# jackbaggins/RayTracing2-fork

Hardware: AMD Instinct MI355X
Metric: Msamples/sec at 1920×1080 Cornell+OBJ; per-pixel RMSE vs CPU ref (higher is better)
Workload: dtype f32

## Files before the change

raytracing2-fork_amd/csrc/device/rt2_k5_resident.h:

```cpp
#pragma once

extern "C" __device__ int rt2_writelane(int value, int lane, int old) __asm("llvm.amdgcn.writelane.i32");

namespace {

constexpr int kResGroups = 38;

struct K5Resident {
    h8 rec[kResGroups * 4 * 64];
};

template <MfmaSpec S>
__device__ __forceinline__ bool exact_group(unsigned long long M, int G, int n_tris, cfloat* tri, const f3& o,
                                            const f3& d, float& best, int& bi, float& bestK, MfmaDiag& dg) {
    if constexpr (S.diag) dg.hot += 1;
    uint32_t m32 = (uint32_t)(M | M >> 32);
    const float bk0 = bestK;
    while (m32) {
        const int tt = __builtin_ctz(m32);
        m32 &= m32 - 1;
        const int idx = 32 * G + tt;
        if (idx >= n_tris) break;
        if constexpr (S.diag) dg.exact += 1;
        cfloat* tp = tri + 12 * idx;
// ... 170 lines not shown
    }
    if constexpr (S.diag) xl_counts(dg, pairs, pairs, (tested + 31) >> 5);
    if (more && __ballot(bestK != bk0)) {
        if constexpr (S.diag) tc = __builtin_amdgcn_s_memtime();
        rebuild();
        if constexpr (S.diag) dg.t_pub += __builtin_amdgcn_s_memtime() - tc;
    }
}

template <MfmaSpec S>
__device__ __forceinline__ void phase_prio(int phase) {
    if constexpr (S.phase_prio > 0) {
        const bool hi = (S.phase_prio == 1 && phase == 0) || (S.phase_prio == 2 && phase == 1) ||
                        (S.phase_prio == 3 && phase == 2) || (S.phase_prio == 4 && phase != 0);
        if (hi)
            __builtin_amdgcn_s_setprio(1);
        else
            __builtin_amdgcn_s_setprio(0);
    }
}

struct ClusterDiag {
    unsigned long long skipped = 0, one = 0, two = 0, rays = 0;
};

__device__ __forceinline__ h8 cluster_rows_frag(const h8* a0, unsigned long long need) {
    typedef uint32_t u4 __attribute__((ext_vector_type(4)));
    const int l = (int)lane_id();
    const int c0 = __popc((uint32_t)need), c1 = __popc((uint32_t)(need >> 32));
    const int rk = (int)lanes_below(need);
    const bool nb = (need >> l) & 1ull;
    const int rest = ((l - rk) + (l < 32 ? c0 : c1 + 2 * c0)) & 31;
    const uint32_t row = (uint32_t)(nb ? rk : rest);
    const auto sw = __builtin_amdgcn_permlane32_swap(row, row, false, false);
    const int half = l & 32;
    const int to0 = 4 * ((int)sw[0] + half), to1 = 4 * ((int)sw[1] + half);
    const u4 b0 = __builtin_bit_cast(u4, a0[0]), b1 = __builtin_bit_cast(u4, a0[1]);
    const bool first = (l & 31) < c0;
    u4 r;
#pragma unroll
    for (int k = 0; k < 4; k++) {
        const int x0 = __builtin_amdgcn_ds_permute(to0, (int)b0[k]);
        const int x1 = __builtin_amdgcn_ds_permute(to1, (int)b1[k]);
        r[k] = (uint32_t)(first ? x0 : x1);
    }
    return __builtin_bit_cast(h8, r);
}

template <MfmaSpec S>
__device__ __forceinline__ bool sweep_kt_res(const RenderParams& p, const h8* rec, const f3& o, const f3& d,
                                             float& best, int& bi, float& bestK, MfmaDiag& dg, bool upper,
                                             unsigned long long act = 0, ClusterDiag* cd = nullptr) {
    const int lane = (int)lane_id();
    [[maybe_unused]] unsigned long long tc = 0, tsw = 0;
    if constexpr (S.diag) tsw = tc = __builtin_amdgcn_s_memtime();
    auto stamp = [&](unsigned long long& acc) {
        if constexpr (S.diag) {
            const unsigned long long t = __builtin_amdgcn_s_memtime();
            acc += t - tc;
            tc = t;
        }
    };
    const f3 m = cross(d, o);
    MfmaScale sc;
    if (!mfma_scale<true>(p.mfma_A, o, d, m, sc)) return false;
    h8 a0[2], y1[2];
    _Float16 tw16;
    kt_frags<S.kt_lane_w>(d, m, sc, a0, tw16);
    constexpr bool per_group = S.exact_win == 1 && !S.y_skip_last && !S.diag;
// ... 86 lines not shown
                            }
                        }
                        auto one_block = [&](const h8& af, int j, int j1) {
                            for (; j + 1 < j1; j += 2) {
                                const h8* t = tb;
                                unsigned long long M0, M1;
                                kt_group_one2(af, t[0], t[64], t[128], t[kKtOps * 64], t[kKtOps * 64 + 64],
                                              t[kKtOps * 64 + 128], M0, M1);
                                const uint32_t m0 = (uint32_t)(M0 | M0 >> 32), m1 = (uint32_t)(M1 | M1 >> 32);
                                maskv = rt2_writelane((int)m0, j, maskv);
                                maskv = rt2_writelane((int)m1, j + 1, maskv);
                                any |= m0 | m1;
                                tb += 2 * kKtOps * 64;
                            }
                            if (j < j1) {
                                const h8 b0 = tb[0], b1 = tb[64], b2 = tb[128], b3 = {};
                                const unsigned long long M = kt_group<false>(&af, y1, b0, b1, b2, b3, false);
                                const uint32_t m32 = (uint32_t)(M | M >> 32);
                                maskv = rt2_writelane((int)m32, j, maskv);
                                any |= m32;
                                tb += kKtOps * 64;
                            }
                        };
#pragma nounroll
                        for (int k = 0; k < ncl; k++) {
                            const int g0 = __float_as_int(ct[8 * k + 3]), gf = __float_as_int(ct[8 * k + 7]);
                            const int g1 = gf & 0xffff;
                            const unsigned long long need =
                                (unsigned long long)(uint32_t)__builtin_amdgcn_readlane(maskv, kNeedLane + 2 * k) |
                                (unsigned long long)(uint32_t)__builtin_amdgcn_readlane(maskv, kNeedLane + 2 * k + 1) << 32;
                            const int c = __popcll(need);
                            const bool compact = (gf & RT2_CLUSTER_COMPACT) != 0;
                            if constexpr (S.diag)
                                if (compact) {
                                    cd->rays += (unsigned long long)c;
                                    if (!c)
                                        cd->skipped += 1;
                                    else if (!upper || c <= 32)
                                        cd->one += 1;
                                    else
                                        cd->two += 1;
                                }
                            if (!c) {
                                tb += (g1 - g0) * (kKtOps * 64);
                                continue;
                            }
                            if (upper && !(compact && c <= 32)) {
                                int up = 1;
                                asm volatile("" : "+s"(up));
                                two_block(g0, g1, up != 0);
                            } else {
                                h8 af = a0[0];
                                if (upper) af = cluster_rows_frag(a0, need);
                                one_block(af, g0, g1);
                            }
                        }
                        maskv = lane < kNeedLane ? maskv : 0;
                    }
                }
            } else {
                for (int j = 0; j < cnt; j++) {
                    const h8 b0 = tb[0], b1 = tb[64], b2 = tb[128];
                    h8 b3 = {};
                    if constexpr (YP) b3 = tb[192];
                    tb += kKtOps * 64;
                    const unsigned long long M = kt_group<YP>(a0, y1, b0, b1, b2, b3, upper);
                    const uint32_t m32 = (uint32_t)(M | M >> 32);
                    if constexpr (W > 1) maskv = lane == j ? (int)m32 : maskv;
                    any |= m32;
// ... 239 lines not shown
        if (lane_id() == 0) {
            atomicAdd(p.seg_counter + 1, dg.groups);
            atomicAdd(p.seg_counter + 2, dg.hot);
            atomicAdd(p.seg_counter + 3, dg.exact);
            atomicAdd(p.seg_counter + 12, dg.t_wait);
            atomicAdd(p.seg_counter + 13, dg.t_filt);
            atomicAdd(p.seg_counter + 14, dg.t_exact);
            atomicAdd(p.seg_counter + 15, dg.t_swp);
            atomicAdd(p.seg_counter + 16, __builtin_amdgcn_s_memtime() - wl_c0);
            atomicAdd(p.seg_counter + 17, dg.t_issue);
            atomicAdd(p.seg_counter + 18, dg.t_pub);
            atomicAdd(p.seg_counter + 19, dg.claims);
            atomicAdd(p.seg_counter + 7, dg.xl[0]);
            atomicAdd(p.seg_counter + 8, dg.xl[1]);
            atomicAdd(p.seg_counter + 9, dg.xl[2]);
            atomicMax(p.seg_counter + 10, dg.xl[3]);
            atomicAdd(p.seg_counter + 22, pds.d.new_ray);
            atomicAdd(p.seg_counter + 23, pds.d.new_px);
            if constexpr (S.cluster_rows) {
                atomicAdd(p.seg_counter + 24, cdg.skipped);
                atomicAdd(p.seg_counter + 25, cdg.one);
                atomicAdd(p.seg_counter + 26, cdg.two);
                atomicAdd(p.seg_counter + 27, cdg.rays);
            }
        }
}

}
```

raytracing2-fork_amd/csrc/device/rt2_mfma.h:

```cpp
#pragma once

namespace {

typedef _Float16 h8 __attribute__((ext_vector_type(8)));
typedef float f4v __attribute__((ext_vector_type(4)));
typedef float f16v __attribute__((ext_vector_type(16)));

constexpr int kMfmaQ = 5;
constexpr float kMfmaC = 1.0009765625f;
constexpr float kMfmaTs = 0x1p-12f;
constexpr float kMfmaB = 2.0f;

struct MfmaSpec {
    int block;
    int waves;
    int tail_lanes;
    bool diag = false;
    int tile_groups = 0;
    bool fair_prio = false;
    int phase_prio = 0;
    bool flow_prio = false;
    bool kt_lane_w = false;
    bool lean = false;
    bool res_l2 = false;
    int exact_win = 1;
    bool y_skip_last = false;
    bool y_first = false;
    bool exact_lanes = false;
    bool pair_loop = false;
    bool cam_park = false;
    bool cluster_rows = false;
};

struct MfmaDiag {
    unsigned long long groups = 0, hot = 0, exact = 0;
    unsigned long long xl[4] = {};
    unsigned long long t_wait = 0, t_filt = 0, t_exact = 0, t_swp = 0;
    unsigned long long unused1 = 0;
    unsigned long long t_issue = 0, t_pub = 0, claims = 0;
};

struct MfmaCoef {
    double c[kMfmaQ][10];
    double tau;
};
__device__ __forceinline__ void mfma_coefs(const float4* tri, int i, int n, MfmaCoef& k, uint32_t* flags) {
    for (int q = 0; q < kMfmaQ; q++)
        for (int c = 0; c < 10; c++) k.c[q][c] = 0.0;
    k.tau = 1.0;
    if (i >= n) {
        k.c[3][9] = 0x1p13;
        return;
    }
    const float4 t0 = tri[3 * i], t1 = tri[3 * i + 1], t2 = tri[3 * i + 2];
// ... 422 lines not shown
#pragma unroll
    for (int i = 0; i < 16; i++)
        t0[i] = __builtin_amdgcn_bitop3_b32(__float_as_int(U0[i]), __float_as_int(V0[i]), __float_as_int(X0[i]), 0x80);
    const f16v U1 = __builtin_amdgcn_mfma_f32_32x32x16_f16(a, bu1, zero, 0, 0, 0);
#pragma unroll
    for (int i = 0; i < 8; i++) acc0 = __builtin_amdgcn_bitop3_b32(t0[2 * i], t0[2 * i + 1], acc0, 0xFE);
    const f16v V1 = __builtin_amdgcn_mfma_f32_32x32x16_f16(a, bv1, zero, 0, 0, 0);
    const f16v X1 = __builtin_amdgcn_mfma_f32_32x32x16_f16(a, bx1, zero, 0, 0, 0);
#pragma unroll
    for (int i = 0; i < 16; i++)
        t1[i] = __builtin_amdgcn_bitop3_b32(__float_as_int(U1[i]), __float_as_int(V1[i]), __float_as_int(X1[i]), 0x80);
#pragma unroll
    for (int i = 0; i < 8; i++) acc1 = __builtin_amdgcn_bitop3_b32(t1[2 * i], t1[2 * i + 1], acc1, 0xFE);
    __builtin_amdgcn_sched_group_barrier(0x008, 3, 0);
    __builtin_amdgcn_sched_group_barrier(0x002, 16, 0);
    __builtin_amdgcn_sched_group_barrier(0x008, 1, 0);
    __builtin_amdgcn_sched_group_barrier(0x002, 8, 0);
    __builtin_amdgcn_sched_group_barrier(0x008, 2, 0);
    __builtin_amdgcn_sched_group_barrier(0x002, 24, 0);
    M0 = __ballot(acc0 < 0);
    M1 = __ballot(acc1 < 0);
}

__device__ __forceinline__ bool sweep_k16(const RenderParams& p, MfmaK16LaneLds& sh, const f3& o, const f3& d,
                                          float& best, int& bi, float& bestK, bool upper) {
    const int lane = (int)lane_id();
    const int r32 = lane & 31, hl = lane >> 5;
    const f3 m = cross(d, o);
    MfmaScale sc;
    if (!mfma_scale<false>(p.mfma_A, o, d, m, sc)) return false;
    mfma_main_row(&sh.ray[lane][0], d, m, o, sc.sigma);
    const float vz = m.z * sc.sigma;
    const _Float16 hz = (_Float16)vz;
    const _Float16 lz = (_Float16)(vz - (float)hz);
    const float zhi = wave_max(fabsf((float)hz));
    const float zlo = wave_max(fabsf((float)lz));
    auto write_y = [&](float bkv) {
        _Float16 s[16];
        mfma_y_chunk(s, d, o, bkv, sc.sigma, sc.Bmax);
        h8* row = reinterpret_cast<h8*>(&sh.ray[lane][32]);
        row[0] = h8{s[0], s[1], s[2], s[3], s[4], s[5], s[6], s[7]};
        row[1] = h8{s[8], s[9], s[10], s[11], s[12], s[13], s[14], s[15]};
    };
    write_y(bestK);
    __builtin_amdgcn_fence(__ATOMIC_RELEASE, "wavefront");
    __builtin_amdgcn_wave_barrier();
// ... 245 lines not shown
    ri[1] = sc.sigma;
    ri[2] = sc.Tw;
    ri[3] = sc.Bmax;
    ri[4] = m.x;
    ri[5] = m.y;
    ri[6] = m.z;
    ri[7] = bestK;
    if (!ok) return;
    mfma_main_row(&sh.ray[lane][0], d, m, o, sc.sigma);
    {
        _Float16 s[16];
        mfma_y_chunk(s, d, o, bestK, sc.sigma, sc.Bmax);
        for (int j = 0; j < 16; j++) sh.ray[lane][32 + j] = s[j];
    }
    __syncthreads();
    for (int j = 0; j < 48; j++) frags[ray * 80 + j] = sh.ray[lane][j];
    const size_t ray0 = (size_t)blockIdx.x * 64;
    if constexpr (kPerm) {
        const int r32 = lane & 31, hl = lane >> 5;
        h8 a0[2], y1[2];
        [[maybe_unused]] ThrBits tb = {};
        [[maybe_unused]] _Float16 tw16 = (_Float16)0.0f;
        if constexpr (kKthr) {
            kt_frags<LAYOUT == 6>(d, m, sc, a0, tw16);
            kt_y(d, o, bestK, sc, tw16, y1);
        } else {
            _Float16 s[18];
            mfma_main_half_slots(s, d, m, sc.sigma);
            frag_pair(s, a0);
            _Float16 t[16];
            mfma_y_chunk(t, d, o, bestK, sc.sigma, sc.Bmax);
            frag_pair(t, y1);
            const float vz = m.z * sc.sigma;
            const _Float16 hz = (_Float16)vz;
            const _Float16 lz = (_Float16)(vz - (float)hz);
            tb = mfma_thr_bits(sc.Tw, wave_max(fabsf((float)lz)), wave_max(fabsf((float)hz)));
        }
        for (int R = 0; R < 2; R++)
            for (int j = 0; j < 8; j++) {
                frags[(ray0 + 32 * R + r32) * 80 + 48 + 8 * hl + j] = a0[R][j];
                frags[(ray0 + 32 * R + r32) * 80 + 64 + 8 * hl + j] = y1[R][j];
            }
        const h8* fg = reinterpret_cast<const h8*>(kKthr ? p.mfma_kt_frag : p.mfma_k16_frag) + lane;
        const int nops = kKthr ? kKtOps : kK16Ops;
        const f16v zero = {};
        for (int G = 0; G < n_pad / 32; G++) {
            h8 b[kK16Ops];
            for (int op = 0; op < nops; op++) b[op] = fg[(size_t)G * nops * 64 + 64 * op];
            for (int R = 0; R < 2; R++) {
                K16Terms q;
                if constexpr (kKthr) {
                    q.U = __builtin_amdgcn_mfma_f32_32x32x16_f16(a0[R], b[0], zero, 0, 0, 0);
                    q.V = __builtin_amdgcn_mfma_f32_32x32x16_f16(a0[R], b[1], zero, 0, 0, 0);
                    q.X = __builtin_amdgcn_mfma_f32_32x32x16_f16(a0[R], b[2], zero, 0, 0, 0);
                    q.T = zero;
                    q.Y = __builtin_amdgcn_mfma_f32_32x32x16_f16(y1[R], b[3], zero, 0, 0, 0);
                } else {
                    const f16v c = __builtin_amdgcn_mfma_f32_32x32x16_f16(mfma_thr_frag(tb), b[6], zero, 0, 0, 0);
                    q.U = __builtin_amdgcn_mfma_f32_32x32x16_f16(a0[R], b[0], c, 0, 0, 0);
                    q.V = __builtin_amdgcn_mfma_f32_32x32x16_f16(a0[R], b[2], c, 0, 0, 0);
                    q.X = __builtin_amdgcn_mfma_f32_32x32x16_f16(a0[R], b[4], c, 0, 0, 0);
                    q.T = c;
                    q.Y = __builtin_amdgcn_mfma_f32_32x32x16_f16(y1[R], b[6], c, 0, 0, 0);
                }
                for (int i = 0; i < 16; i++) {
                    const size_t rr = ray0 + 32 * R + 8 * (i >> 2) + 4 * hl + (i & 3);
                    float* tt = terms + (rr * n_pad + 32 * G + r32) * 5;
                    tt[0] = q.U[i];
// ... 80 lines not shown
```

raytracing2-fork_amd/csrc/device/rt2_render.hip:

```cpp
#include <hip/hip_runtime.h>

#include <algorithm>
#include <cstdio>
#include <cstdlib>
#include <cstring>
#include <mutex>
#include <string>
#include <type_traits>
#include <vector>

#include "../../../include/rt2.h"
#include "../../../include/rt2_cluster.h"
#include "rt2_math.h"

using namespace rt2d;

#include "rt2_sweep.h"
#include "rt2_path.h"
#include "rt2_brute.h"
#include "rt2_mfma.h"
#include "rt2_k5_tiles.h"
#include "rt2_k5_resident.h"
#include "rt2_assist.h"
#include "rt2_bvh.h"
// ... 368 lines not shown
        HIPCHECK(hipMalloc(&s->d_mfma_k16, (size_t)n_pad32 * kK16Ops * 16 * sizeof(_Float16)));
        HIPCHECK(hipMalloc(&s->d_mfma_k16_tau, (size_t)n_pad32 * sizeof(float)));
        HIPCHECK(hipMalloc(&s->d_mfma_k16_bnd, (size_t)n_pad32 * sizeof(float2)));
        uint32_t* d_mflags = reinterpret_cast<uint32_t*>(s->d_counters + kCounters - 2);
        HIPCHECK(hipMemset(d_mflags, 0, 2 * sizeof(uint32_t)));
        hipLaunchKernelGGL(prep_mfma_k16, dim3((n_pad32 + 255) / 256), dim3(256), 0, 0, s->d_tri, n_tris, n_pad32,
                           s->d_mfma_k16, s->d_mfma_k16_tau, s->d_mfma_k16_bnd, d_mflags);
        HIPCHECK(hipGetLastError());
        uint32_t mflags[2];
        HIPCHECK(hipMemcpy(mflags, d_mflags, sizeof(mflags), hipMemcpyDeviceToHost));
        HIPCHECK(hipMemset(d_mflags, 0, 2 * sizeof(uint32_t)));
        std::memcpy(&s->mfma_A, &mflags[1], sizeof(float));
        s->mfma_ok = s->mfma_A <= 0x1p20f;
        const size_t kt_bytes = (size_t)n_pad32 * kKtOps * 16 * sizeof(_Float16);
        if (n_pad32 / 32 <= kResGroups && rt2_cluster_table_build(tris, n_tris, &s->clusters) < 0) return -1;
        HIPCHECK(hipMalloc(&s->d_mfma_kt, kt_bytes + sizeof(s->clusters)));
        HIPCHECK(hipMemcpy(reinterpret_cast<char*>(s->d_mfma_kt) + kt_bytes, &s->clusters, sizeof(s->clusters),
                           hipMemcpyHostToDevice));
        hipLaunchKernelGGL(prep_mfma_kt, dim3((n_pad32 + 255) / 256), dim3(256), 0, 0, s->d_tri, n_tris, n_pad32,
                           s->d_mfma_kt, d_mflags);
        HIPCHECK(hipGetLastError());
        HIPCHECK(hipDeviceSynchronize());
        HIPCHECK(hipMemset(d_mflags, 0, 2 * sizeof(uint32_t)));
    }
    HIPCHECK(hipDeviceSynchronize());
    return 0;
}

static int ensure_mfma16(rt2_scene* s) {
    if (s->d_mfma || s->n_tris <= 0) return 0;
    HIPCHECK(hipSetDevice(s->device));
    const int n_pad = (s->n_tris + 15) / 16 * 16;
    HIPCHECK(hipMalloc(&s->d_mfma, (size_t)n_pad * kMfmaQ * 32 * sizeof(_Float16)));
    HIPCHECK(hipMalloc(&s->d_mfma_tau, (size_t)n_pad * sizeof(float)));
    HIPCHECK(hipDeviceSynchronize());
    uint32_t* d_mflags = reinterpret_cast<uint32_t*>(s->d_counters + kCounters - 2);
    HIPCHECK(hipMemset(d_mflags, 0, 2 * sizeof(uint32_t)));
    hipLaunchKernelGGL(prep_mfma, dim3((n_pad + 255) / 256), dim3(256), 0, 0, s->d_tri, s->n_tris, n_pad, s->d_mfma,
                       s->d_mfma_tau, d_mflags);
    HIPCHECK(hipGetLastError());
    HIPCHECK(hipMemset(d_mflags, 0, 2 * sizeof(uint32_t)));
    HIPCHECK(hipDeviceSynchronize());
    return 0;
}

extern "C" void rt2_scene_destroy(rt2_scene* s) {
// ... 101 lines not shown
}
#ifdef RT2_EXPERIMENTS
constexpr MfmaSpec kt_yw(MfmaSpec x) {
    x.y_first = true;
    return x;
}
#endif
constexpr MfmaSpec kt_xl(MfmaSpec x) {
    x.exact_lanes = true;
    return x;
}
constexpr MfmaSpec kt_pair(MfmaSpec x) {
    x.pair_loop = true;
    return x;
}
constexpr MfmaSpec kt_park(MfmaSpec x) {
    x.cam_park = true;
    return x;
}
constexpr MfmaSpec kt_cr(MfmaSpec x) {
    x.cluster_rows = true;
    return x;
}
constexpr int kResWin = 38;
constexpr int kResL2Groups = 256;
constexpr MfmaSpec kt_tiles_flow() {
    return MfmaSpec{.block = 768, .waves = 3, .tail_lanes = 0, .tile_groups = 19, .flow_prio = true, .kt_lane_w = true};
}
constexpr MfmaSpec kt_tiles_flow4() {
    MfmaSpec x = kt_tiles_flow();
    x.block = 1024;
    x.waves = 4;
    x.lean = true;
    return x;
}
constexpr Bvh3Spec kBvhDefault{.block = 256, .thresh = 16, .slab = Slab::Markstein, .waves = 5, .diag = false};

#ifdef RT2_EXPERIMENTS
constexpr SmemSpec smem_x(int g, Filter f, Tail t, int lanes, int w, bool stats = false) {
    return SmemSpec{.block = 256, .group = g, .filter = f, .tail = t, .tail_lanes = lanes, .waves = w, .stats = stats};
}
constexpr SplitSpec split_x(int s, Filter f, int w) {
    return SplitSpec{.waves_per_ray = s, .group = 8, .filter = f, .waves = w};
}
constexpr Bvh3Spec bvh3_x(int t, Slab sl, int w, bool diag = false) {
    return Bvh3Spec{.block = 256, .thresh = t, .slab = sl, .waves = w, .diag = diag};
}
#endif

constexpr Variant kVariants[] = {
    RT2_VARIANT(0, K_SMEM, render_smem<kSmemDefault>, 256, "smem/256/max3f8/coop32/w6/lockstep"),
    RT2_VARIANT(109, K_BVH4, render_bvh4<kBvhDefault>, 256, "bvh4/256/t16/w5"),
    RT2_VARIANT(86, K_TILED, render_tiled<kTiledLarge>, 512, "tiled/512/max3f4"),
    RT2_VARIANT(92, K_ASSIST, render_assist<kAssist12>, 768, "assist12/max3f8/w6"),
    RT2_VARIANT(136, K_SMEM, render_smem<kSmemDefault>, 256, "smem/256/max3f8/coop32/w6/lockstep"),
    RT2_VARIANT(227, K_MFMA, render_mfma<kMfmaK5>, 256, "mfma/256/k5/coop8/w3/imax/minred/ymma/t12/llds/ser4/cmp"),
    RT2_VARIANT(353, K_MFMA, render_mfma_k5r<kt_cr(kt_park(kt_pair(kt_xl(kt_win(kt_res(false, false, true, 4), kResWin)))))>, 1024, "mfmar/1024/kt4/res38/coop4/w4/cmp/dpp/lean/lw/pp4", kResGroups),
    RT2_VARIANT(354, K_MFMA, render_mfma_k5r<kt_cr(kt_park(kt_pair(kt_xl(kt_win(kt_res(false, true, true), kResWin)))))>, 1024, "mfmar/1024/kt4/res38/coop4/w4/cmp/fair/dpp/lean/lw", kResGroups),
    RT2_VARIANT(355, K_MFMA, render_mfma_k5r<kt_win(kt_res(true, false, true, 4), kResWin)>, 1024, "mfmarl2/1024/kt4/res38l2/coop4/w4/cmp/dpp/lean/lw/pp4", kResL2Groups),
    RT2_VARIANT(356, K_MFMA, render_mfma_k5r<kt_win(kt_res(true, true, true), kResWin)>, 1024, "mfmarl2/1024/kt4/res38l2/coop4/w4/cmp/fair/dpp/lean/lw", kResL2Groups),
    RT2_VARIANT(380, K_MFMA, render_mfma_k5t<kt_tiles_flow4()>, 1024, "mfmat5/1024/kt4/tile19/coop0/w4/cmp/regs/perm/lw/flowp/lean"),
#ifdef RT2_EXPERIMENTS
    RT2_VARIANT(342, K_MFMA, render_mfma_k5r<kt_win(kt_res(false, false, false), kResWin)>, 1024, "mfmar/1024/kt4/res38/coop4/w4/cmp/dpp/lean", kResGroups),
    RT2_VARIANT(344, K_MFMA, render_mfma_k5r<kt_win(kt_res(false, true, false), kResWin)>, 1024, "mfmar/1024/kt4/res38/coop4/w4/cmp/fair/dpp/lean", kResGroups),
    RT2_VARIANT(345, K_MFMA, render_mfma_k5r<kt_win(kt_res(true, false, false), kResWin)>, 1024, "mfmarl2/1024/kt4/res38l2/coop4/w4/cmp/dpp/lean", kResL2Groups),
    RT2_VARIANT(346, K_MFMA, render_mfma_k5r<kt_win(kt_res(true, true, false), kResWin)>, 1024, "mfmarl2/1024/kt4/res38l2/coop4/w4/cmp/fair/dpp/lean", kResL2Groups),
    RT2_VARIANT(387, K_MFMA, render_mfma_k5r<kt_win(kt_res(false, false, true, 1), kResWin)>, 1024, "mfmar/1024/kt4/res38/coop4/w4/cmp/dpp/lean/lw/pp1", kResGroups),
    RT2_VARIANT(388, K_MFMA, render_mfma_k5r<kt_win(kt_res(false, false, true, 2), kResWin)>, 1024, "mfmar/1024/kt4/res38/coop4/w4/cmp/dpp/lean/lw/pp2", kResGroups),
    RT2_VARIANT(389, K_MFMA, render_mfma_k5r<kt_win(kt_res(false, false, true, 3), kResWin)>, 1024, "mfmar/1024/kt4/res38/coop4/w4/cmp/dpp/lean/lw/pp3", kResGroups),
    RT2_VARIANT(391, K_MFMA, render_mfma_k5r<kt_win(kt_res(false, false, true), kResWin)>, 1024, "mfmar/1024/kt4/res38/coop4/w4/cmp/dpp/lean/lw", kResGroups),
    RT2_VARIANT(350, K_MFMA, render_mfma_k5r<kt_win(kt_res(false, false, true, 0, true), kResWin)>, 1024, "mfmar/1024/kt4/res38/coop4/w4/cmp/diag/dpp/lean/lw", kResGroups),
    RT2_VARIANT(390, K_MFMA, render_mfma_k5r<kt_win(kt_res(false, false, true, 0, true), 1)>, 1024, "mfmar/1024/kt4/res38/coop4/w4/cmp/diag/dpp/lean/lw/xw1", kResGroups),
    RT2_VARIANT(392, K_MFMA, render_mfma_k5r<kt_win(kt_res(false, false, true, 4), 1)>, 1024, "mfmar/1024/kt4/res38/coop4/w4/cmp/dpp/lean/lw/pp4/xw1", kResGroups),
    RT2_VARIANT(393, K_MFMA, render_mfma_k5r<kt_win(kt_res(false, false, true, 4), 1, true)>, 1024, "mfmar/1024/kt4/res38/coop4/w4/cmp/dpp/lean/lw/pp4/xw1s", kResGroups),
    RT2_VARIANT(394, K_MFMA, render_mfma_k5r<kt_win(kt_res(false, false, true, 4), 2)>, 1024, "mfmar/1024/kt4/res38/coop4/w4/cmp/dpp/lean/lw/pp4/xw2", kResGroups),
    RT2_VARIANT(395, K_MFMA, render_mfma_k5r<kt_win(kt_res(false, false, true, 4), 4)>, 1024, "mfmar/1024/kt4/res38/coop4/w4/cmp/dpp/lean/lw/pp4/xw4", kResGroups),
    RT2_VARIANT(396, K_MFMA, render_mfma_k5r<kt_win(kt_res(false, false, true, 4), 8)>, 1024, "mfmar/1024/kt4/res38/coop4/w4/cmp/dpp/lean/lw/pp4/xw8", kResGroups),
    RT2_VARIANT(399, K_MFMA, render_mfma_k5r<kt_win(kt_res(false, false, true, 4), 19)>, 1024, "mfmar/1024/kt4/res38/coop4/w4/cmp/dpp/lean/lw/pp4/xw19", kResGroups),
    RT2_VARIANT(397, K_MFMA, render_mfma_k5r<kt_win(kt_res(true, false, true, 4), 1)>, 1024, "mfmarl2/1024/kt4/res38l2/coop4/w4/cmp/dpp/lean/lw/pp4/xw1", kResL2Groups),
    RT2_VARIANT(398, K_MFMA, render_mfma_k5r<kt_win(kt_res(false, true, true), 1)>, 1024, "mfmar/1024/kt4/res38/coop4/w4/cmp/fair/dpp/lean/lw/xw1", kResGroups),
    RT2_VARIANT(351, K_MFMA, render_mfma_k5r<kt_yw(kt_win(kt_res(false, false, true, 4), kResWin))>, 1024, "mfmar/1024/kt4/res38/coop4/w4/cmp/dpp/lean/lw/pp4/yw", kResGroups),
    RT2_VARIANT(352, K_MFMA, render_mfma_k5r<kt_yw(kt_win(kt_res(true, false, true, 4), kResWin))>, 1024, "mfmarl2/1024/kt4/res38l2/coop4/w4/cmp/dpp/lean/lw/pp4/yw", kResL2Groups),
    RT2_VARIANT(357, K_MFMA, render_mfma_k5r<kt_yw(kt_win(kt_res(false, false, true, 0, true), kResWin))>, 1024, "mfmar/1024/kt4/res38/coop4/w4/cmp/diag/dpp/lean/lw/yw", kResGroups),
    RT2_VARIANT(400, K_MFMA, render_mfma_k5r<kt_win(kt_res(false, false, true, 4), kResWin)>, 1024, "mfmar/1024/kt4/res38/coop4/w4/cmp/dpp/lean/lw/pp4/xwave", kResGroups),
    RT2_VARIANT(401, K_MFMA, render_mfma_k5r<kt_xl(kt_win(kt_res(true, false, true, 4), kResWin))>, 1024, "mfmarl2/1024/kt4/res38l2/coop4/w4/cmp/dpp/lean/lw/pp4/xl", kResL2Groups),
    RT2_VARIANT(402, K_MFMA, render_mfma_k5r<kt_xl(kt_win(kt_res(false, false, true, 0, true), kResWin))>, 1024, "mfmar/1024/kt4/res38/coop4/w4/cmp/diag/dpp/lean/lw/xl", kResGroups),
    RT2_VARIANT(403, K_MFMA, render_mfma_k5r<kt_win(kt_res(false, true, true), kResWin)>, 1024, "mfmar/1024/kt4/res38/coop4/w4/cmp/fair/dpp/lean/lw/xwave", kResGroups),
    RT2_VARIANT(404, K_MFMA, render_mfma_k5r<kt_xl(kt_win(kt_res(true, true, true), kResWin))>, 1024, "mfmarl2/1024/kt4/res38l2/coop4/w4/cmp/fair/dpp/lean/lw/xl", kResL2Groups),
    RT2_VARIANT(405, K_MFMA, render_mfma_k5r<kt_xl(kt_win(kt_res(false, false, true, 4), kResWin))>, 1024, "mfmar/1024/kt4/res38/coop4/w4/cmp/dpp/lean/lw/pp4/nopair/nopark", kResGroups),
    RT2_VARIANT(406, K_MFMA, render_mfma_k5r<kt_pair(kt_xl(kt_win(kt_res(false, false, true, 4), kResWin)))>, 1024, "mfmar/1024/kt4/res38/coop4/w4/cmp/dpp/lean/lw/pp4/nopark", kResGroups),
    RT2_VARIANT(407, K_MFMA, render_mfma_k5r<kt_park(kt_xl(kt_win(kt_res(false, false, true, 4), kResWin)))>, 1024, "mfmar/1024/kt4/res38/coop4/w4/cmp/dpp/lean/lw/pp4/nopair", kResGroups),
    RT2_VARIANT(408, K_MFMA, render_mfma_k5r<kt_xl(kt_win(kt_res(false, true, true), kResWin))>, 1024, "mfmar/1024/kt4/res38/coop4/w4/cmp/fair/dpp/lean/lw/nopair/nopark", kResGroups),
    RT2_VARIANT(409, K_MFMA, render_mfma_k5r<kt_park(kt_pair(kt_xl(kt_win(kt_res(false, false, true, 4), kResWin))))>, 1024, "mfmar/1024/kt4/res38/coop4/w4/cmp/dpp/lean/lw/pp4/nocr", kResGroups),
    RT2_VARIANT(410, K_MFMA, render_mfma_k5r<kt_park(kt_pair(kt_xl(kt_win(kt_res(false, true, true), kResWin))))>, 1024, "mfmar/1024/kt4/res38/coop4/w4/cmp/fair/dpp/lean/lw/nocr", kResGroups),
    RT2_VARIANT(411, K_MFMA, render_mfma_k5r<kt_cr(kt_pair(kt_xl(kt_win(kt_res(false, false, true, 0, true), kResWin))))>, 1024, "mfmar/1024/kt4/res38/coop4/w4/cmp/diag/dpp/lean/lw/xl/cr", kResGroups),
    RT2_VARIANT(370, K_MFMA, render_mfma_k5t<kt_tiles_flow()>, 768, "mfmat5/768/kt4/tile19/coop0/w3/cmp/regs/perm/lw/flowp"),
    RT2_VARIANT(368, K_MFMA, render_mfma_k5t<[] { MfmaSpec x = kt_tiles_flow(); x.diag = true; return x; }()>, 768, "mfmat5/768/kt4/tile19/coop0/w3/cmp/regs/perm/lw/flowp/diag"),
    RT2_VARIANT(369, K_MFMA, render_mfma_k5t<[] { MfmaSpec x = kt_tiles_flow(); x.flow_prio = false; return x; }()>, 768, "mfmat5/768/kt4/tile19/coop0/w3/cmp/regs/perm/lw/flow"),
    RT2_VARIANT(382, K_MFMA, render_mfma_k5t<[] { MfmaSpec x = kt_tiles_flow(); x.lean = true; return x; }()>, 768, "mfmat5/768/kt4/tile19/coop0/w3/cmp/regs/perm/lw/flowp/lean"),
    RT2_VARIANT(381, K_MFMA, render_mfma_k5t<[] { MfmaSpec x = kt_tiles_flow4(); x.tile_groups = 16; return x; }()>, 1024, "mfmat5/1024/kt4/tile16/coop0/w4/cmp/regs/perm/lw/flowp/lean"),
    RT2_VARIANT(385, K_MFMA, render_mfma_k5t<[] { MfmaSpec x = kt_tiles_flow4(); x.flow_prio = false; return x; }()>, 1024, "mfmat5/1024/kt4/tile19/coop0/w4/cmp/regs/perm/lw/flow/lean"),
    RT2_VARIANT(386, K_MFMA, render_mfma_k5t<[] { MfmaSpec x = kt_tiles_flow4(); x.tail_lanes = 4; return x; }()>, 1024, "mfmat5/1024/kt4/tile19/coop4/w4/cmp/regs/perm/lw/flowp/lean"),
    RT2_VARIANT(67, K_SMEM, render_smem<kSmemMid>, 256, "smem/256/max3f8/coop32"),
    RT2_VARIANT(85, K_SPLIT, render_split<kSplitSmall>, 256, "split4/max3f8/w6"),
    RT2_VARIANT(53, K_BVH3, render_bvh3<kBvhDefault>, 256, "bvh3/256/t16/w5"),
    RT2_VARIANT(106, K_SMEM, render_smem<kSmemFree>, 256, "smem/256/max3f8/coop32/w6/free"),
    RT2_VARIANT(37, K_BVH, render_bvh<BvhSpec{256}>, 256, "bvh/256"),
    RT2_VARIANT(40, K_BVH2, (render_bvh2<Bvh2Spec{256, 16}>), 256, "bvh2/256/t16"),
    RT2_VARIANT(41, K_BVH2, (render_bvh2<Bvh2Spec{256, 8}>), 256, "bvh2/256/t8"),
    RT2_VARIANT(43, K_BVH2, (render_bvh2<Bvh2Spec{128, 16}>), 128, "bvh2/128/t16"),
    RT2_VARIANT(45, K_BVH2, (render_bvh2<Bvh2Spec{256, 1}>), 256, "bvh2/256/t1"),
    RT2_VARIANT(46, K_BVH3, render_bvh3<bvh3_x(16, Slab::Markstein, 1)>, 256, "bvh3/256/t16"),
    RT2_VARIANT(47, K_BVH3, render_bvh3<bvh3_x(8, Slab::Markstein, 1)>, 256, "bvh3/256/t8"),
    RT2_VARIANT(48, K_BVH3, render_bvh3<bvh3_x(24, Slab::Markstein, 1)>, 256, "bvh3/256/t24"),
    RT2_VARIANT(50, K_BVH3, render_bvh3<bvh3_x(16, Slab::Binary64, 1)>, 256, "bvh3/256/t16/div64"),
    RT2_VARIANT(54, K_BVH3, render_bvh3<bvh3_x(8, Slab::Markstein, 5)>, 256, "bvh3/256/t8/w5"),
    RT2_VARIANT(55, K_BVH3, render_bvh3<bvh3_x(16, Slab::Filtered, 5)>, 256, "bvh3/256/t16/filt/w5"),
    RT2_VARIANT(58, K_BVH3, render_bvh3<bvh3_x(16, Slab::Markstein, 5, true)>, 256, "bvh3/256/t16/w5/DIAG"),
// ... 982 lines not shown
    bool ok = t->n >= 0 && t->n <= RT2_MAX_CLUSTERS && (t->n == 0 || ng <= kResGroups) && t->far_o >= 0.0f;
    int g = 0;
    for (int k = 0; ok && k < t->n; k++) {
        const int g1 = t->c[k].g1_flags & 0xffff;
        ok = t->c[k].g0 == g && g1 > g && (t->c[k].g1_flags & ~(0xffff | RT2_CLUSTER_COMPACT)) == 0;
        g = g1;
    }
    if (!ok || (t->n > 0 && g != ng)) {
        rt2h::set_error("rt2_scene_set_clusters: the ranges must be contiguous and cover the scene's groups");
        return -1;
    }
    HIPCHECK(hipSetDevice(s->device));
    HIPCHECK(hipDeviceSynchronize());
    s->clusters = *t;
    const size_t kt_bytes = (size_t)ng * 32 * kKtOps * 16 * sizeof(_Float16);
    HIPCHECK(hipMemcpy(reinterpret_cast<char*>(s->d_mfma_kt) + kt_bytes, &s->clusters, sizeof(s->clusters),
                       hipMemcpyHostToDevice));
    return 0;
}

extern "C" int rt2_mfma_probe(rt2_scene* s, int layout, const float* rays, int32_t n_rays, float* terms,
                              uint16_t* frags, float* rinfo, uint8_t* accept) {
    if (!s || !rays || n_rays <= 0 || n_rays % 64 != 0 || !terms || !frags || !rinfo || !accept ||
        layout < 0 || layout > 6 || s->n_tris < 1 || !s->mfma_ok) {
        rt2h::set_error("rt2_mfma_probe: bad argument (n_rays a positive multiple of 64, a scene in the filter's "
                        "range)");
        return -1;
    }
    HIPCHECK(hipSetDevice(s->device));
    if (layout == 0 && ensure_mfma16(s) != 0) return -1;
    const int n_pad = layout >= 1 ? (s->n_tris + 31) / 32 * 32 : (s->n_tris + 15) / 16 * 16;
    const size_t nr = (size_t)n_rays;
    const size_t b_rays = nr * 8 * sizeof(float), b_terms = nr * n_pad * 5 * sizeof(float),
                 b_frags = nr * 80 * sizeof(uint16_t), b_info = nr * 8 * sizeof(float), b_acc = nr * s->n_tris;
    char* d = nullptr;
    HIPCHECK(hipMalloc(&d, b_rays + b_terms + b_frags + b_info + b_acc + 64));
    char* p0 = d;
    float4* d_rays = (float4*)p0;
    float* d_terms = (float*)(p0 += b_rays);
    _Float16* d_frags = (_Float16*)(p0 += b_terms);
    float* d_info = (float*)(p0 += b_frags);
    uint8_t* d_acc = (uint8_t*)(p0 += b_info);
    int rc = 0;
    auto run = [&]() -> int {
        HIPCHECK(hipMemcpy(d_rays, rays, b_rays, hipMemcpyHostToDevice));
        HIPCHECK(hipMemset(d_terms, 0, b_terms));
        RenderParams p;
        std::memset(&p, 0, sizeof(p));
        p.tri = s->d_tri;
        p.n_tris = s->n_tris;
        p.mfma_frag = s->d_mfma;
        p.mfma_tau = s->d_mfma_tau;
        p.mfma_A = s->mfma_A;
        p.mfma_k16_frag = s->d_mfma_k16;
        p.mfma_k16_tau = s->d_mfma_k16_tau;
        p.mfma_k16_bnd = s->d_mfma_k16_bnd;
        p.mfma_kt_frag = s->d_mfma_kt;
        const auto launch = [&](auto kernel) {
            hipLaunchKernelGGL(kernel, dim3(n_rays / 64), dim3(64), 0, 0, p, d_rays, n_pad, d_terms, d_frags, d_info,
                               d_acc);
        };
        switch (layout) {
        case 0: launch(mfma_probe_kernel<0>); break;
        case 1: launch(mfma_probe_kernel<1>); break;
        case 2: launch(mfma_probe_kernel<2>); break;
        case 3: launch(mfma_probe_kernel<3>); break;
        case 4: launch(mfma_probe_kernel<4>); break;
        case 5: launch(mfma_probe_kernel<5>); break;
        default: launch(mfma_probe_kernel<6>); break;
        }
        HIPCHECK(hipGetLastError());
        HIPCHECK(hipDeviceSynchronize());
        HIPCHECK(hipMemcpy(terms, d_terms, b_terms, hipMemcpyDeviceToHost));
        HIPCHECK(hipMemcpy(frags, d_frags, b_frags, hipMemcpyDeviceToHost));
        HIPCHECK(hipMemcpy(rinfo, d_info, b_info, hipMemcpyDeviceToHost));
        HIPCHECK(hipMemcpy(accept, d_acc, b_acc, hipMemcpyDeviceToHost));
        return 0;
    };
    rc = run();
    (void)hipFree(d);
    return rc;
}
```

Before: 1645.

## Use 16x16x32 MFMA path for compact clusters needing at most sixteen rays

Adds a cluster_rows16 mode that compacts the rays needing a compact cluster into 16 rows and runs the triangle filter with 16x16x32 f16 MFMAs split into low and high halves, instead of the 32-row path. It also adds a matching probe layout, a diagnostic counter, and a host check that disables the MFMA path when the fragment records contain inf/nan. The intent is to cut MFMA work and latency for sparse clusters. The cost is extra permlane and ds_permute shuffles, plus a different code path whose scheduling barriers may interact poorly with the existing pipeline.

```diff
diff --git a/raytracing2-fork_amd/csrc/device/rt2_k5_resident.h b/raytracing2-fork_amd/csrc/device/rt2_k5_resident.h
--- a/raytracing2-fork_amd/csrc/device/rt2_k5_resident.h
+++ b/raytracing2-fork_amd/csrc/device/rt2_k5_resident.h
@@ -216,6 +216,7 @@
 
 struct ClusterDiag {
     unsigned long long skipped = 0, one = 0, two = 0, rays = 0;
+    unsigned long long r16 = 0;
 };
 
 __device__ __forceinline__ h8 cluster_rows_frag(const h8* a0, unsigned long long need) {
@@ -239,6 +240,33 @@
         r[k] = (uint32_t)(first ? x0 : x1);
     }
     return __builtin_bit_cast(h8, r);
+}
+
+__device__ __forceinline__ void cluster_rows_frag16(const h8* a0, unsigned long long need, h8& alo, h8& ahi) {
+    typedef uint32_t u4 __attribute__((ext_vector_type(4)));
+    const int l = (int)lane_id();
+    const int c0 = __popc((uint32_t)need), c1 = __popc((uint32_t)(need >> 32));
+    const int rk = (int)lanes_below(need);
+    const bool nb = (need >> l) & 1ull;
+    const int rest = ((l - rk) + (l < 32 ? c0 : c1 + 2 * c0)) & 31;
+    const uint32_t row = (uint32_t)(nb ? rk : rest);
+    const uint32_t dst = row + (row & 16);
+    const auto sw = __builtin_amdgcn_permlane32_swap(dst, dst, false, false);
+    const int half = (l & 32) >> 1;
+    const int to0 = 4 * ((int)sw[0] + half), to1 = 4 * ((int)sw[1] + half);
+    const u4 b0 = __builtin_bit_cast(u4, a0[0]), b1 = __builtin_bit_cast(u4, a0[1]);
+    const bool first = (l & 15) < c0, low = l < 32;
+    u4 rl, rh;
+#pragma unroll
+    for (int k = 0; k < 4; k++) {
+        const int x0 = __builtin_amdgcn_ds_permute(to0, (int)b0[k]);
+        const int x1 = __builtin_amdgcn_ds_permute(to1, (int)b1[k]);
+        const uint32_t q = (uint32_t)(first ? x0 : x1);
+        rl[k] = low ? q : 0u;
+        rh[k] = __builtin_amdgcn_permlane32_swap(0u, q, false, false)[0];
+    }
+    alo = __builtin_bit_cast(h8, rl);
+    ahi = __builtin_bit_cast(h8, rh);
 }
 
 template <MfmaSpec S>
@@ -371,6 +399,26 @@
                                 tb += kKtOps * 64;
                             }
                         };
+                        [[maybe_unused]] auto one_block16 = [&](const h8& alo, const h8& ahi, int j, int j1) {
+                            const int d16 = kt16_record_lane(lane) - lane;
+                            const h8* t = tb + d16;
+                            for (; j + 1 < j1; j += 2) {
+                                uint32_t m0, m1;
+                                kt_group16_2(alo, ahi, t[0], t[64], t[128], t[kKtOps * 64], t[kKtOps * 64 + 64],
+                                             t[kKtOps * 64 + 128], m0, m1);
+                                maskv = rt2_writelane((int)m0, j, maskv);
+                                maskv = rt2_writelane((int)m1, j + 1, maskv);
+                                any |= m0 | m1;
+                                t += 2 * kKtOps * 64;
+                            }
+                            if (j < j1) {
+                                const uint32_t m32 = kt_group16(alo, ahi, t[0], t[64], t[128]);
+                                maskv = rt2_writelane((int)m32, j, maskv);
+                                any |= m32;
+                                t += kKtOps * 64;
+                            }
+                            tb = t - d16;
+                        };
 #pragma nounroll
                         for (int k = 0; k < ncl; k++) {
                             const int g0 = __float_as_int(ct[8 * k + 3]), gf = __float_as_int(ct[8 * k + 7]);
@@ -389,11 +437,19 @@
                                         cd->one += 1;
                                     else
                                         cd->two += 1;
+                                    if (c && c <= 16) cd->r16 += 1;
                                 }
                             if (!c) {
                                 tb += (g1 - g0) * (kKtOps * 64);
                                 continue;
                             }
+                            if constexpr (S.cluster_rows16)
+                                if (compact && c <= 16) {
+                                    h8 alo, ahi;
+                                    cluster_rows_frag16(a0, need, alo, ahi);
+                                    one_block16(alo, ahi, g0, g1);
+                                    continue;
+                                }
                             if (upper && !(compact && c <= 32)) {
                                 int up = 1;
                                 asm volatile("" : "+s"(up));
@@ -679,8 +735,9 @@
                 atomicAdd(p.seg_counter + 25, cdg.one);
                 atomicAdd(p.seg_counter + 26, cdg.two);
                 atomicAdd(p.seg_counter + 27, cdg.rays);
-            }
-        }
-}
-
-}
+                atomicAdd(p.seg_counter + 28, cdg.r16);
+            }
+        }
+}
+
+}
diff --git a/raytracing2-fork_amd/csrc/device/rt2_mfma.h b/raytracing2-fork_amd/csrc/device/rt2_mfma.h
--- a/raytracing2-fork_amd/csrc/device/rt2_mfma.h
+++ b/raytracing2-fork_amd/csrc/device/rt2_mfma.h
@@ -30,6 +30,7 @@
     bool pair_loop = false;
     bool cam_park = false;
     bool cluster_rows = false;
+    bool cluster_rows16 = false;
 };
 
 struct MfmaDiag {
@@ -498,6 +499,63 @@
     M1 = __ballot(acc1 < 0);
 }
 
+__device__ __forceinline__ int kt16_record_lane(int l) { return (l & 15) + 16 * (l >> 5) + 32 * ((l >> 4) & 1); }
+__device__ __forceinline__ int kt16_fold(const f4v& U, const f4v& V, const f4v& X) {
+    int t[4];
+#pragma unroll
+    for (int i = 0; i < 4; i++)
+        t[i] = __builtin_amdgcn_bitop3_b32(__float_as_int(U[i]), __float_as_int(V[i]), __float_as_int(X[i]), 0x80);
+    return __builtin_amdgcn_bitop3_b32(t[0], t[1], t[2], 0xFE) | t[3];
+}
+__device__ __forceinline__ uint32_t kt16_hot(unsigned long long Mlo, unsigned long long Mhi) {
+    const uint32_t lo = (uint32_t)(Mlo | Mlo >> 32), hi = (uint32_t)(Mhi | Mhi >> 32);
+    return ((lo | lo >> 16) & 0xffffu) | (hi | hi >> 16) << 16;
+}
+__device__ __forceinline__ uint32_t kt_group16(const h8& alo, const h8& ahi, const h8& bu, const h8& bv,
+                                               const h8& bx) {
+    const f4v zero = {};
+    const f4v Ul = __builtin_amdgcn_mfma_f32_16x16x32_f16(alo, bu, zero, 0, 0, 0);
+    const f4v Vl = __builtin_amdgcn_mfma_f32_16x16x32_f16(alo, bv, zero, 0, 0, 0);
+    const f4v Xl = __builtin_amdgcn_mfma_f32_16x16x32_f16(alo, bx, zero, 0, 0, 0);
+    const f4v Uh = __builtin_amdgcn_mfma_f32_16x16x32_f16(ahi, bu, zero, 0, 0, 0);
+    const f4v Vh = __builtin_amdgcn_mfma_f32_16x16x32_f16(ahi, bv, zero, 0, 0, 0);
+    const f4v Xh = __builtin_amdgcn_mfma_f32_16x16x32_f16(ahi, bx, zero, 0, 0, 0);
+    const int al = kt16_fold(Ul, Vl, Xl);
+    const int ah = kt16_fold(Uh, Vh, Xh);
+    __builtin_amdgcn_sched_group_barrier(0x008, 6, 0);
+    __builtin_amdgcn_sched_group_barrier(0x002, 12, 0);
+    return kt16_hot(__ballot(al < 0), __ballot(ah < 0));
+}
+__device__ __forceinline__ void kt_group16_2(const h8& alo, const h8& ahi, const h8& bu0, const h8& bv0,
+                                             const h8& bx0, const h8& bu1, const h8& bv1, const h8& bx1, uint32_t& m0,
+                                             uint32_t& m1) {
+    const f4v zero = {};
+    const f4v Ul0 = __builtin_amdgcn_mfma_f32_16x16x32_f16(alo, bu0, zero, 0, 0, 0);
+    const f4v Vl0 = __builtin_amdgcn_mfma_f32_16x16x32_f16(alo, bv0, zero, 0, 0, 0);
+    const f4v Xl0 = __builtin_amdgcn_mfma_f32_16x16x32_f16(alo, bx0, zero, 0, 0, 0);
+    const f4v Uh0 = __builtin_amdgcn_mfma_f32_16x16x32_f16(ahi, bu0, zero, 0, 0, 0);
+    const f4v Vh0 = __builtin_amdgcn_mfma_f32_16x16x32_f16(ahi, bv0, zero, 0, 0, 0);
+    const f4v Xh0 = __builtin_amdgcn_mfma_f32_16x16x32_f16(ahi, bx0, zero, 0, 0, 0);
+    const int al0 = kt16_fold(Ul0, Vl0, Xl0);
+    const f4v Ul1 = __builtin_amdgcn_mfma_f32_16x16x32_f16(alo, bu1, zero, 0, 0, 0);
+    const f4v Vl1 = __builtin_amdgcn_mfma_f32_16x16x32_f16(alo, bv1, zero, 0, 0, 0);
+    const f4v Xl1 = __builtin_amdgcn_mfma_f32_16x16x32_f16(alo, bx1, zero, 0, 0, 0);
+    const int ah0 = kt16_fold(Uh0, Vh0, Xh0);
+    const f4v Uh1 = __builtin_amdgcn_mfma_f32_16x16x32_f16(ahi, bu1, zero, 0, 0, 0);
+    const f4v Vh1 = __builtin_amdgcn_mfma_f32_16x16x32_f16(ahi, bv1, zero, 0, 0, 0);
+    const f4v Xh1 = __builtin_amdgcn_mfma_f32_16x16x32_f16(ahi, bx1, zero, 0, 0, 0);
+    const int al1 = kt16_fold(Ul1, Vl1, Xl1);
+    const int ah1 = kt16_fold(Uh1, Vh1, Xh1);
+    __builtin_amdgcn_sched_group_barrier(0x008, 6, 0);
+    __builtin_amdgcn_sched_group_barrier(0x002, 6, 0);
+    __builtin_amdgcn_sched_group_barrier(0x008, 3, 0);
+    __builtin_amdgcn_sched_group_barrier(0x002, 6, 0);
+    __builtin_amdgcn_sched_group_barrier(0x008, 3, 0);
+    __builtin_amdgcn_sched_group_barrier(0x002, 12, 0);
+    m0 = kt16_hot(__ballot(al0 < 0), __ballot(ah0 < 0));
+    m1 = kt16_hot(__ballot(al1 < 0), __ballot(ah1 < 0));
+}
+
 __device__ __forceinline__ bool sweep_k16(const RenderParams& p, MfmaK16LaneLds& sh, const f3& o, const f3& d,
                                           float& best, int& bi, float& bestK, bool upper) {
     const int lane = (int)lane_id();
@@ -789,7 +847,7 @@
         [[maybe_unused]] ThrBits tb = {};
         [[maybe_unused]] _Float16 tw16 = (_Float16)0.0f;
         if constexpr (kKthr) {
-            kt_frags<LAYOUT == 6>(d, m, sc, a0, tw16);
+            kt_frags<LAYOUT >= 6>(d, m, sc, a0, tw16);
             kt_y(d, o, bestK, sc, tw16, y1);
         } else {
             _Float16 s[18];
@@ -811,6 +869,38 @@
         const h8* fg = reinterpret_cast<const h8*>(kKthr ? p.mfma_kt_frag : p.mfma_k16_frag) + lane;
         const int nops = kKthr ? kKtOps : kK16Ops;
         const f16v zero = {};
+        if constexpr (LAYOUT == 7) {
+            typedef uint32_t u4 __attribute__((ext_vector_type(4)));
+            const h8* fg16 = reinterpret_cast<const h8*>(p.mfma_kt_frag) + kt16_record_lane(lane);
+            const f4v zero4 = {};
+            for (int R16 = 0; R16 < 4; R16++) {
+                const u4 src = __builtin_bit_cast(u4, a0[R16 >> 1]);
+                u4 lo, hi;
+                for (int k = 0; k < 4; k++) {
+                    const uint32_t v = (uint32_t)__shfl((int)src[k], 16 * (R16 & 1) + (lane & 15) + 32 * ((lane >> 4) & 1));
+                    lo[k] = lane < 32 ? v : 0u;
+                    hi[k] = lane < 32 ? 0u : v;
+                }
+                const h8 alo = __builtin_bit_cast(h8, lo), ahi = __builtin_bit_cast(h8, hi);
+                for (int G = 0; G < n_pad / 32; G++) {
+                    const h8* t = fg16 + (size_t)G * kKtOps * 64;
+                    f4v q[2][3];
+                    for (int op = 0; op < 3; op++) {
+                        q[0][op] = __builtin_amdgcn_mfma_f32_16x16x32_f16(alo, t[64 * op], zero4, 0, 0, 0);
+                        q[1][op] = __builtin_amdgcn_mfma_f32_16x16x32_f16(ahi, t[64 * op], zero4, 0, 0, 0);
+                    }
+                    for (int h = 0; h < 2; h++)
+                        for (int i = 0; i < 4; i++) {
+                            const size_t rr = ray0 + 16 * R16 + 4 * (lane >> 4) + i;
+                            float* tt = terms + (rr * n_pad + 32 * G + 16 * h + (lane & 15)) * 5;
+                            tt[0] = q[h][0][i];
+                            tt[1] = q[h][1][i];
+                            tt[2] = q[h][2][i];
+                        }
+                }
+            }
+            return;
+        }
         for (int G = 0; G < n_pad / 32; G++) {
             h8 b[kK16Ops];
             for (int op = 0; op < nops; op++) b[op] = fg[(size_t)G * nops * 64 + 64 * op];
diff --git a/raytracing2-fork_amd/csrc/device/rt2_render.hip b/raytracing2-fork_amd/csrc/device/rt2_render.hip
--- a/raytracing2-fork_amd/csrc/device/rt2_render.hip
+++ b/raytracing2-fork_amd/csrc/device/rt2_render.hip
@@ -414,6 +414,12 @@
         HIPCHECK(hipGetLastError());
         HIPCHECK(hipDeviceSynchronize());
         HIPCHECK(hipMemset(d_mflags, 0, 2 * sizeof(uint32_t)));
+        if (s->mfma_ok && n_pad32 / 32 <= kResGroups) {
+            std::vector<uint16_t> rec(kt_bytes / sizeof(uint16_t));
+            HIPCHECK(hipMemcpy(rec.data(), s->d_mfma_kt, kt_bytes, hipMemcpyDeviceToHost));
+            for (uint16_t h : rec)
+                if ((h & 0x7c00u) == 0x7c00u) s->mfma_ok = 0;
+        }
     }
     HIPCHECK(hipDeviceSynchronize());
     return 0;
@@ -561,6 +567,11 @@
     x.cluster_rows = true;
     return x;
 }
+constexpr MfmaSpec kt_cr16(MfmaSpec x) {
+    x.cluster_rows = true;
+    x.cluster_rows16 = true;
+    return x;
+}
 constexpr int kResWin = 38;
 constexpr int kResL2Groups = 256;
 constexpr MfmaSpec kt_tiles_flow() {
@@ -594,8 +605,8 @@
     RT2_VARIANT(92, K_ASSIST, render_assist<kAssist12>, 768, "assist12/max3f8/w6"),
     RT2_VARIANT(136, K_SMEM, render_smem<kSmemDefault>, 256, "smem/256/max3f8/coop32/w6/lockstep"),
     RT2_VARIANT(227, K_MFMA, render_mfma<kMfmaK5>, 256, "mfma/256/k5/coop8/w3/imax/minred/ymma/t12/llds/ser4/cmp"),
-    RT2_VARIANT(353, K_MFMA, render_mfma_k5r<kt_cr(kt_park(kt_pair(kt_xl(kt_win(kt_res(false, false, true, 4), kResWin)))))>, 1024, "mfmar/1024/kt4/res38/coop4/w4/cmp/dpp/lean/lw/pp4", kResGroups),
-    RT2_VARIANT(354, K_MFMA, render_mfma_k5r<kt_cr(kt_park(kt_pair(kt_xl(kt_win(kt_res(false, true, true), kResWin)))))>, 1024, "mfmar/1024/kt4/res38/coop4/w4/cmp/fair/dpp/lean/lw", kResGroups),
+    RT2_VARIANT(353, K_MFMA, render_mfma_k5r<kt_cr16(kt_park(kt_pair(kt_xl(kt_win(kt_res(false, false, true, 4), kResWin)))))>, 1024, "mfmar/1024/kt4/res38/coop4/w4/cmp/dpp/lean/lw/pp4", kResGroups),
+    RT2_VARIANT(354, K_MFMA, render_mfma_k5r<kt_cr16(kt_park(kt_pair(kt_xl(kt_win(kt_res(false, true, true), kResWin)))))>, 1024, "mfmar/1024/kt4/res38/coop4/w4/cmp/fair/dpp/lean/lw", kResGroups),
     RT2_VARIANT(355, K_MFMA, render_mfma_k5r<kt_win(kt_res(true, false, true, 4), kResWin)>, 1024, "mfmarl2/1024/kt4/res38l2/coop4/w4/cmp/dpp/lean/lw/pp4", kResL2Groups),
     RT2_VARIANT(356, K_MFMA, render_mfma_k5r<kt_win(kt_res(true, true, true), kResWin)>, 1024, "mfmarl2/1024/kt4/res38l2/coop4/w4/cmp/fair/dpp/lean/lw", kResL2Groups),
     RT2_VARIANT(380, K_MFMA, render_mfma_k5t<kt_tiles_flow4()>, 1024, "mfmat5/1024/kt4/tile19/coop0/w4/cmp/regs/perm/lw/flowp/lean"),
@@ -632,7 +643,9 @@
     RT2_VARIANT(408, K_MFMA, render_mfma_k5r<kt_xl(kt_win(kt_res(false, true, true), kResWin))>, 1024, "mfmar/1024/kt4/res38/coop4/w4/cmp/fair/dpp/lean/lw/nopair/nopark", kResGroups),
     RT2_VARIANT(409, K_MFMA, render_mfma_k5r<kt_park(kt_pair(kt_xl(kt_win(kt_res(false, false, true, 4), kResWin))))>, 1024, "mfmar/1024/kt4/res38/coop4/w4/cmp/dpp/lean/lw/pp4/nocr", kResGroups),
     RT2_VARIANT(410, K_MFMA, render_mfma_k5r<kt_park(kt_pair(kt_xl(kt_win(kt_res(false, true, true), kResWin))))>, 1024, "mfmar/1024/kt4/res38/coop4/w4/cmp/fair/dpp/lean/lw/nocr", kResGroups),
-    RT2_VARIANT(411, K_MFMA, render_mfma_k5r<kt_cr(kt_pair(kt_xl(kt_win(kt_res(false, false, true, 0, true), kResWin))))>, 1024, "mfmar/1024/kt4/res38/coop4/w4/cmp/diag/dpp/lean/lw/xl/cr", kResGroups),
+    RT2_VARIANT(411, K_MFMA, render_mfma_k5r<kt_cr16(kt_pair(kt_xl(kt_win(kt_res(false, false, true, 0, true), kResWin))))>, 1024, "mfmar/1024/kt4/res38/coop4/w4/cmp/diag/dpp/lean/lw/xl/cr16", kResGroups),
+    RT2_VARIANT(412, K_MFMA, render_mfma_k5r<kt_cr(kt_park(kt_pair(kt_xl(kt_win(kt_res(false, false, true, 4), kResWin)))))>, 1024, "mfmar/1024/kt4/res38/coop4/w4/cmp/dpp/lean/lw/pp4/cr32", kResGroups),
+    RT2_VARIANT(413, K_MFMA, render_mfma_k5r<kt_cr(kt_park(kt_pair(kt_xl(kt_win(kt_res(false, true, true), kResWin)))))>, 1024, "mfmar/1024/kt4/res38/coop4/w4/cmp/fair/dpp/lean/lw/cr32", kResGroups),
     RT2_VARIANT(370, K_MFMA, render_mfma_k5t<kt_tiles_flow()>, 768, "mfmat5/768/kt4/tile19/coop0/w3/cmp/regs/perm/lw/flowp"),
     RT2_VARIANT(368, K_MFMA, render_mfma_k5t<[] { MfmaSpec x = kt_tiles_flow(); x.diag = true; return x; }()>, 768, "mfmat5/768/kt4/tile19/coop0/w3/cmp/regs/perm/lw/flowp/diag"),
     RT2_VARIANT(369, K_MFMA, render_mfma_k5t<[] { MfmaSpec x = kt_tiles_flow(); x.flow_prio = false; return x; }()>, 768, "mfmat5/768/kt4/tile19/coop0/w3/cmp/regs/perm/lw/flow"),
@@ -1661,7 +1674,7 @@
 extern "C" int rt2_mfma_probe(rt2_scene* s, int layout, const float* rays, int32_t n_rays, float* terms,
                               uint16_t* frags, float* rinfo, uint8_t* accept) {
     if (!s || !rays || n_rays <= 0 || n_rays % 64 != 0 || !terms || !frags || !rinfo || !accept ||
-        layout < 0 || layout > 6 || s->n_tris < 1 || !s->mfma_ok) {
+        layout < 0 || layout > 7 || s->n_tris < 1 || !s->mfma_ok) {
         rt2h::set_error("rt2_mfma_probe: bad argument (n_rays a positive multiple of 64, a scene in the filter's "
                         "range)");
         return -1;
@@ -1706,7 +1719,8 @@
         case 3: launch(mfma_probe_kernel<3>); break;
         case 4: launch(mfma_probe_kernel<4>); break;
         case 5: launch(mfma_probe_kernel<5>); break;
-        default: launch(mfma_probe_kernel<6>); break;
+        case 6: launch(mfma_probe_kernel<6>); break;
+        default: launch(mfma_probe_kernel<7>); break;
         }
         HIPCHECK(hipGetLastError());
         HIPCHECK(hipDeviceSynchronize());
```

Result: faster. 1731 (median of 6 runs) (+5.3%).
